# LeonOrou/OPF-Graph-Neural-Solver

Measured on AMD Instinct MI355X. Metric: grids/sec (fwd+bwd) on batched case118, K=4, higher is better.
Workload: dtype f32

## Files before the change

### opf-graph-neural-solver_amd/csrc/gns_backward_split.hip

```cpp
#include "gns_device.h"
#include "gns_kernels.h"
#include "gns_dw.h"
#include "gns_phys_device.h"

typedef int gns_i8v __attribute__((ext_vector_type(8)));
#ifndef GNS_BWDS_ONE_LAYOUT
#define GNS_BWDS_ONE_LAYOUT 0
#endif
#ifndef GNS_BWDS_WPE
#define GNS_BWDS_WPE 2
#endif
#ifndef GNS_BWDS_KEEP_SLOPES
#define GNS_BWDS_KEEP_SLOPES 1
#endif
#if GNS_BWDS_KEEP_SLOPES
#define GNS_SLOPES(sl) sl
#define GNS_SLOPE_OF(sl, layer, act, u) sl[layer][u]
#else
#define GNS_SLOPES(sl) nullptr
#define GNS_SLOPE_OF(sl, layer, act, u) dlrelu2(act[u])
#endif
#ifndef GNS_BWDS_FRESH_INPUTS
#define GNS_BWDS_FRESH_INPUTS 1
#endif
#define GNS_BWDS_PHYS_THREADS (GNS_BWDS_PHYS_WAVES * 64)

__global__ void __launch_bounds__(GNS_BWDS_PHYS_THREADS) gns_bwds_phys_kernel(GnsBwdsArgs A) {
  extern __shared__ __attribute__((aligned(16))) float lds[];
  constexpr int W = GNS_BWDS_PHYS_WAVES;
  const int lane = threadIdx.x & 63;
  const int wave = __builtin_amdgcn_readfirstlane(threadIdx.x >> 6);
  const int N = A.N, E = A.E, K = A.K, k = A.k;
  cip topo = (cip)A.topo;
  const long long g = blockIdx.x;
  long long b = g * GNS_LANES + lane;
  bool live = b < A.Bt;
  if (A.group_topo) {
    const int s = A.slot_grid[g * GNS_LANES + lane];
    b = s;
    live = s >= 0 && s < A.Bt;
    if (!gns_group_topo(A.topo, A.group_topo, g, N, E, topo)) return;
  }
  constexpr int pidx = 4;
  static_assert(GNS_BWDS_PHYS_WAVES == 16, "pidx");
  const cip in_ptr = topo + topo[TH_IN_PTR], out_ptr = topo + topo[TH_OUT_PTR], q2p = topo + topo[TH_Q2P], is_gen = topo + topo[TH_IS_GEN],
            incd_ptr = topo + topo[TH_INCD_PTR], incd = topo + topo[TH_INCD],
            part = topo + topo[TH_PART] + pidx * (GNS_MAXP + 1), epart = topo + topo[TH_EPART] + pidx * (GNS_MAXP + 1);
  const int n0 = part[wave], n1 = part[wave + 1];
  const int e0 = epart[wave], e1 = epart[wave + 1];
  const bool use_plane = A.use_plane != 0, plane_dp = A.use_plane == 2;
  float* const red = lds;
  float* const pl_v = lds + W * GNS_LANES;
  float* const pl_th = pl_v + (use_plane ? N * GNS_LANES : 0);
  float* const pl_dp = pl_th + (plane_dp ? N * GNS_LANES : 0);
  const long long R = gns_in_rows(N, E);
  const float* IN = A.in;
  const long long in_base = g * R, row_ein = in_base + 3LL * N, row_eout = row_ein + 3LL * E, row_grid = row_eout + E;
  const float gt = (live && A.g_total) ? A.g_total[b] : 0.f;
  const float gl = (live && A.g_last) ? A.g_last[b] : 0.f;
  const int RB = A.RB, RBA = A.RBA;
  auto state_row = [&](int slot, int n) { return (((long long)slot * A.G + g) * N + n) * RB; };
  auto adj_row = [&](int n) { return (g * N + n) * RBA; };
  auto slot_ptr = [&](int j, int p) { return A.slots + ((g * 6 + j) * E + p) * GNS_LANES + lane; };
  const f4 gsum = *row_ptr(IN, row_grid, lane);
  const float invN = 1.0f / (float)N;
  const bool last = k == K - 1;
  const int mode = A.mode;
  const bool x2_live = mode == 2 || k + 1 < K - 1;
  const float cdp = 2.f * (gt * A.gwk + (last ? gl : 0.f)) * invN;
  const f2 lamv = reinterpret_cast<const f2*>(A.lam)[((long long)k * A.G + g) * GNS_LANES + lane];
  const int bits = (int)lamv.y;
  const bool low1 = bits & 1, low2 = bits & 2;

  float lb = 0.f;
  constexpr int PB = 4;
  for (int nb = n0; nb < n1; nb += PB) {
    f4 s1[PB], a0[PB], x0[PB], x1[PB], x2[PB], b1[PB];
#pragma unroll
    for (int j = 0; j < PB; ++j) {
      const int n = min(nb + j, n1 - 1);
      const long long ar = adj_row(n);
      s1[j] = *row_ptr(A.state, state_row(k + 1, n), lane);
      b1[j] = *row_ptr(IN, in_base + 3LL * n + 1, lane);
      if (!last) {
        a0[j] = *row_ptr(A.adj, ar, lane);
        x0[j] = *row_ptr(A.adj, ar + (mode == 2 ? 3 : 1), lane);
        x1[j] = *row_ptr(A.adj, ar + (mode == 0 ? 2 : (mode == 2 ? 3 : 1)), lane);
        x2[j] = *row_ptr(A.adj, ar + (x2_live ? 3 : 1), lane);
      }
    }
#pragma unroll
    for (int j = 0; j < PB; ++j) {
      const int n = nb + j;
      if (n < n1) {
        f4 a;
        if (last) {
          const float vb = (live && A.g_v) ? ((s1[j].x < 0.f) ? 0.f : A.g_v[b * N + n]) : 0.f;
          const float tb = (live && A.g_theta) ? A.g_theta[b * N + n] : 0.f;
          a = f4{vb, tb, 0.f, 0.f};
        } else {
          f4 xs;
          if (mode == 2) xs = x2[j];
          else if (mode == 1) xs = x2_live ? f4{x2[j].x + x0[j].x, x2[j].y + x0[j].y, x2[j].z + x0[j].z, 0.f} : x0[j];
          else if (x2_live) xs = f4{(x2[j].x + x0[j].x) + x1[j].x, (x2[j].y + x0[j].y) + x1[j].y, (x2[j].z + x0[j].z) + x1[j].z, 0.f};
          else xs = f4{x0[j].x + x1[j].x, x0[j].y + x1[j].y, x0[j].z + x1[j].z, 0.f};
          a = f4{a0[j].x + xs.x, a0[j].y + xs.y, xs.z, 0.f};
        }
        a.z = a.z + cdp * s1[j].z;
        a.w = 2.f * b1[j].w * s1[j].x;
        *row_ptr(A.adj, adj_row(n), lane) = a;
        if (use_plane) { pl_v[n * GNS_LANES + lane] = s1[j].x; pl_th[n * GNS_LANES + lane] = s1[j].y; }
        if (plane_dp) pl_dp[n * GNS_LANES + lane] = a.z;
        lb += a.z * (low2 ? 2.f * (b1[j].y - b1[j].x) : 2.f * (b1[j].z - b1[j].y));
      }
    }
  }
  red[wave * GNS_LANES + lane] = lb;
  __syncthreads();
  float lbar = 0.f;
#pragma unroll
  for (int w = 0; w < W; ++w) lbar += red[w * GNS_LANES + lane];
  const float pgbar = lbar / (low1 ? 2.f * (gsum.y - gsum.z) : 2.f * (gsum.w - gsum.y));

  {
    const cip erec = topo + topo[TH_EREC];
    struct EdgeIn { f4 e1v, o0; float vs, ths, vt, tht, tha, thb, thc, thd, Fb, Tb; bool gs, gt; };
    auto edge_load = [&](int p, EdgeIn& L) {
      const gns_i8v r = *reinterpret_cast<const __attribute__((address_space(4))) gns_i8v*>(erec + 8 * p);
      const int s = r[0], t = r[1], ia = r[2], ib = r[3], q = r[4], ic = r[5], id = r[6];
      L.gs = is_gen[s] != 0; L.gt = is_gen[t] != 0;
      L.e1v = *row_ptr(IN, row_ein + 3LL * p + 1, lane);
      L.o0 = *row_ptr(IN, row_eout + q, lane);
      if (use_plane) {
        L.vs = pl_v[s * GNS_LANES + lane]; L.ths = pl_th[s * GNS_LANES + lane];
        L.vt = pl_v[t * GNS_LANES + lane]; L.tht = pl_th[t * GNS_LANES + lane];
        L.tha = pl_th[ia * GNS_LANES + lane]; L.thb = pl_th[ib * GNS_LANES + lane];
        L.thc = pl_th[ic * GNS_LANES + lane]; L.thd = pl_th[id * GNS_LANES + lane];
        if (plane_dp) { L.Fb = pl_dp[t * GNS_LANES + lane]; L.Tb = pl_dp[s * GNS_LANES + lane]; }
        else { L.Fb = row_ptr(A.adj, adj_row(t), lane)->z; L.Tb = row_ptr(A.adj, adj_row(s), lane)->z; }
      } else {
        const f4 ss = *row_ptr(A.state, state_row(k + 1, s), lane), st = *row_ptr(A.state, state_row(k + 1, t), lane);
        L.vs = ss.x; L.ths = ss.y; L.vt = st.x; L.tht = st.y;
        L.tha = row_ptr(A.state, state_row(k + 1, ia), lane)->y; L.thb = row_ptr(A.state, state_row(k + 1, ib), lane)->y;
        L.thc = row_ptr(A.state, state_row(k + 1, ic), lane)->y; L.thd = row_ptr(A.state, state_row(k + 1, id), lane)->y;
        L.Fb = row_ptr(A.adj, adj_row(t), lane)->z;
        L.Tb = row_ptr(A.adj, adj_row(s), lane)->z;
      }
    };
    auto edge_adjoint = [&](int p, const EdgeIn& L) {
      const LineTrig T = line_trig<false>(L.ths, L.tht, L.tha, L.thb, L.thc, L.thd, L.e1v.w, L.o0.z);
      const LineAdj R = line_state_adjoint(T, L.vs, L.vt, L.e1v.y, L.e1v.z, L.o0.x, L.o0.y, L.Fb, L.Tb, pgbar);
      if (!L.gs) *slot_ptr(0, p) = R.dvs;
      if (!L.gt) *slot_ptr(1, p) = R.dvt;
      *slot_ptr(2, p) = R.dths;
      *slot_ptr(4, p) = R.dbar; *slot_ptr(5, p) = R.dbar2;
    };
    for (int p = e0; p < e1; p += 2) {
      EdgeIn L0, L1;
      edge_load(p, L0);
      edge_load(min(p + 1, e1 - 1), L1);
      edge_adjoint(p, L0);
      if (p + 1 < e1) edge_adjoint(p + 1, L1);
    }
  }
  __syncthreads();

  for (int n = n0; n < n1; ++n) {
    const long long ar = adj_row(n);
    const f4 a0 = *row_ptr(A.adj, ar, lane);
    float vbar = a0.x, thbar = a0.y;
    const float dpb = a0.z;
    const int p0 = in_ptr[n], p1 = in_ptr[n + 1], q0 = out_ptr[n], q1 = out_ptr[n + 1], i0 = incd_ptr[n], i1 = incd_ptr[n + 1];
    const bool gen = is_gen[n] != 0;
    {
      float ai[4], bi[4], ao[4], bo[4], ci[8];
#pragma unroll
// ... 77 lines not shown
  f32x4 T1[NB1], T2, T4[NT4];
  cfp nb, ptl;

  __device__ __forceinline__ void init(const GnsBwdsArgs& A) {
    const long long koff = A.k;
    nb = (cfp)A.pn + A.n_off[C::NPHI + l] + koff * A.n_sz[C::NPHI + l];
    ptl = (cfp)A.pt + A.t_off[C::NPHI + l] + koff * A.t_sz[C::NPHI + l];
    scalar_cache_warm(ptl, A.t_sz[C::NPHI + l]);
#if !GNS_BWDS_ONE_LAYOUT
    scalar_cache_warm(nb, A.n_sz[C::NPHI + l]);
#endif
    const f32x4 z4 = {0.f, 0.f, 0.f, 0.f};
#pragma unroll
    for (int t = 0; t < NB1; ++t) T1[t] = z4;
#pragma unroll
    for (int t = 0; t < NT4; ++t) T4[t] = z4;
    T2 = z4;
  }

  template <bool ACC_GS, bool STEP0, bool IG = false>
  __device__ __forceinline__ void bus(const GnsBwdsArgs& A, float* rec, int lane, long long g, int n, float g3s, f2 (&xs)[XL],
                                      f2 (&macc)[D / 2], f4& xsum, f2 (&gS)[H / 2]) {
    f2 (&S)[H / 2] = reinterpret_cast<f2 (&)[H / 2]>(xs[SOFF]);
    load_pairs<H>(A.msg, ((((long long)A.k * A.G + g) * A.N + n) * C::NPHI + fphi) * C::HQ, lane, S);
    WFirst wf;
    f2 a1[H / 2], a2[H / 2], g2[H / 2], g1[H / 2];
    f2 sl[2][H / 2];
    using TL [[maybe_unused]] = TLay<LIN, H, OUTP>;
#if GNS_BWDS_ONE_LAYOUT
    (void)wf;
    mlp2_fwd<LIN, H>(ptl, xs, a1, a2, NoBG{}, NoLink{}, GNS_SLOPES(sl));
#else
    using LKm = std::conditional_t<STEP0, NoLink, L2>; using LKs = std::conditional_t<STEP0, std::conditional_t<FOLD4, L0, NoLink>, std::conditional_t<FOLD4, L1, L2>>;
    if constexpr (STEP0) {
      f2 u4[H / 2];
      const f2 (&st)[2] = reinterpret_cast<const f2 (&)[2]>(xs[0]);
      const f2 (&tl)[(LIN - 4 - D + 1) / 2] = reinterpret_cast<const f2 (&)[(LIN - 4 - D + 1) / 2]>(xs[SOFF]);
      phi_head<4, H>(ptl, st, u4);
      phi_tail<LIN, H, 4 + D>(ptl, u4, tl, a1, a2, NoBG{}, NoLink{}, GNS_SLOPES(sl));
    } else {
      mlp2_fwd<LIN, H>(ptl, xs, a1, a2, NoBG{}, L0{nullptr, nb, &wf}, GNS_SLOPES(sl));
    }
#endif
#if GNS_BWDS_ONE_LAYOUT
    if constexpr (l == 2) {
      bwd_rows_fwd_layout<H, OUTP>(ptl + TL::oW4, macc, g2);
    } else {
      const f2 g3v[1] = {f2{g3s, 0.f}};
      bwd_rows_fwd_layout<H, 2>(ptl + TL::oW4, g3v, g2);
    }
#else
    if constexpr (l == 2) {
      bwd_rows<OUTP, H>(nb, macc, g2, NoBG{}, LKm{&wf, nullptr, nullptr});
    } else {
      const f2 g3v[1] = {f2{g3s, 0.f}};
      bwd_rows<2, H>(nb, g3v, g2, NoBG{}, LKs{&wf, nb + NL::oW2, &wf});
    }
#endif
#pragma unroll
    for (int u = 0; u < H / 2; ++u) g2[u] = g2[u] * GNS_SLOPE_OF(sl, 1, a2, u);
    if constexpr (FOLD4 || FOLDM) {
      static_for<0, H / 2>([&](auto j_) { constexpr int j = decltype(j_)::value; gws_putB<SW>(rec, lane, 8 + j, a2[j]); });
      gws_putB<SW>(rec, lane, 8 + H / 2, f2{1.f, 0.f});
      if constexpr (FOLDM) {
        static_for<0, 8>([&](auto j_) { constexpr int j = decltype(j_)::value; gws_putA<SW>(rec, lane, j, macc[j]); });
        gws_w2r(); gws_pass<SW, 16>(rec, lane, T4[0]); gws_r2w();
      }
    } else {
      static_for<0, H / 2>([&](auto j_) { constexpr int j = decltype(j_)::value; gws_putB<SW>(rec, lane, j, a2[j]); });
      gws_putB<SW>(rec, lane, H / 2, f2{1.f, 0.f});
      static_for<0, NA4>([&](auto t_) {
        constexpr int t = decltype(t_)::value;
        if constexpr (l == 2) {
          static_for<0, 6>([&](auto j_) { constexpr int j = decltype(j_)::value; if constexpr (6 * t + j < D / 2) gws_putA<SW>(rec, lane, j, macc[6 * t + j]); });
        } else {
          gws_putA<SW>(rec, lane, 0, f2{g3s, 0.f});
        }
        gws_w2r(); gws_pass<SW>(rec, lane, T4[t]); gws_r2w();
      });
    }
#if GNS_BWDS_ONE_LAYOUT
    bwd_rows_fwd_layout<H, H>(ptl + TL::oW2, g2, g1);
#else
    bwd_rows<H, H>(nb + NL::oW2, g2, g1, NoBG{}, std::conditional_t<FOLD4, L2, NoLink>{&wf, nullptr, nullptr});
#endif
#pragma unroll
    for (int u = 0; u < H / 2; ++u) g1[u] = g1[u] * GNS_SLOPE_OF(sl, 0, a1, u);
    if constexpr (IG && STEP0) {
      float ax[4];
#pragma unroll
      for (int i = 0; i < 4; ++i) {
        float acc = 0.f;
#pragma unroll
        for (int u = 0; u < H / 2; ++u) { acc = fmaf(ptl[i * H + 2 * u], g1[u].x, acc); acc = fmaf(ptl[i * H + 2 * u + 1], g1[u].y, acc); }
        ax[i] = acc;
      }
      xsum.x += ax[0]; xsum.y += ax[1]; xsum.z += ax[2]; xsum.w += ax[3];
    }
    static_for<0, H / 2>([&](auto j_) { constexpr int j = decltype(j_)::value; gws_putA<SW>(rec, lane, j, g2[j]); gws_putB<SW>(rec, lane, j, a1[j]); });
    gws_putB<SW>(rec, lane, H / 2, f2{1.f, 0.f});
    gws_w2r(); gws_pass<SW>(rec, lane, T2); gws_r2w();
    static_for<0, H / 2>([&](auto j_) { constexpr int j = decltype(j_)::value; gws_putA<SW>(rec, lane, j, g1[j]); });
    if constexpr (FOLD4) gws_putA<SW>(rec, lane, H / 2, f2{g3s, 0.f});
    if constexpr (FOLDM) static_for<0, (OUT - 16) / 2>([&](auto j_) { constexpr int j = decltype(j_)::value; gws_putA<SW>(rec, lane, H / 2 + j, macc[8 + j]); });
    static_for<0, NB1>([&](auto t_) {
      constexpr int t = decltype(t_)::value;
      constexpr int po = (WIDE && t == NB1 - 1) ? W2OFF / 2 : 0;
      static_for<0, 8>([&](auto j_) { constexpr int j = decltype(j_)::value; if constexpr (8 * t + j < XL) gws_putB<SW>(rec, lane, po + j, xs[8 * t + j]); });
      gws_w2r(); gws_pass<SW, (WIDE && t == NB1 - 1) ? W2OFF : 0>(rec, lane, T1[t]); gws_r2w();
    });
    auto to_consumers = [&](auto ip_, f2 v) {
      constexpr int ip = decltype(ip_)::value;
      if constexpr (ip == 0) { xsum.x += v.x; xsum.y += v.y; }
      else if constexpr (ip == 1) xsum.z += v.x;
      else if constexpr (ip < SOFF) macc[ip - 2] += v;
      else if constexpr (ip < SOFF + H / 2) { if constexpr (ACC_GS) gS[ip - SOFF] += v; else gS[ip - SOFF] = v; }
    };
#if GNS_BWDS_ONE_LAYOUT
    bwd_from_fwd_layout<2 * (SOFF + H / 2), H, cf16p>(ptl, g1, to_consumers);
#else
    if constexpr (STEP0) {
      constexpr int G0 = (2 * SOFF) / 4, G1 = (2 * SOFF + H - 1) / 4 + 1;
      bwd_inputs<G1 - G0, H>(nb + NL::total + G0 * H * 4, g1, [&](auto ip_, f2 v) {
        constexpr int ip = decltype(ip_)::value + 2 * G0;
        if constexpr (ip >= SOFF && ip < SOFF + H / 2) { if constexpr (ACC_GS) gS[ip - SOFF] += v; else gS[ip - SOFF] = v; }
      });
    } else {
      bwd_inputs<(LIN + 3) / 4, H>(nb + NL::total, g1, to_consumers);
    }
#endif
  }

  __device__ __forceinline__ void flush(const GnsBwdsArgs& A, int lane, float* slab) {
    const long long koff = A.k;
    constexpr int ob1 = LIN * H, oW2 = ob1 + H, ob2 = oW2 + H * H, oW4 = ob2 + H, ob4 = oW4 + OUT * H;
    float* lb_ = slab + A.g_off[C::NPHI + l] + koff * A.g_sz[C::NPHI + l];
    static_for<0, NB1>([&](auto t_) { constexpr int t = decltype(t_)::value;
      gws_flush(lane, T1[t], lb_, [&](int c, int il) {
        const bool lastw = WIDE && t == NB1 - 1;
        const int i = 16 * t + il;
        if (c < H) return (lastw && il >= XT) ? -1 : (i < LIN ? c * LIN + i : (i == LIN ? ob1 + c : -1));
        if (FOLD4 && lastw && c == H && il >= XT && il <= XT + H) return il - XT < H ? oW4 + (il - XT) : ob4;
        if (FOLDM && lastw && c >= H && c < H + (OUT - 16) && il >= XT && il <= XT + H) { const int j = 16 + c - H; return il - XT < H ? oW4 + j * H + (il - XT) : ob4 + j; }
        return -1; }, true); });
    gws_flush(lane, T2, lb_, [&](int c, int il) { return c < H ? (il < H ? oW2 + c * H + il : (il == H ? ob2 + c : -1)) : -1; }, true);
    if constexpr (FOLDM)
      gws_flush(lane, T4[0], lb_, [&](int c, int il) { return il < H ? oW4 + c * H + il : (il == H ? ob4 + c : -1); }, true);
    else if constexpr (!FOLD4)
    static_for<0, NA4>([&](auto t_) { constexpr int t = decltype(t_)::value;
      gws_flush(lane, T4[t], lb_, [&](int c, int il) { const int j = 12 * t + c; return (c < 12 && j < OUT) ? (il < H ? oW4 + j * H + il : (il == H ? ob4 + j : -1)) : -1; }, true); });
  }
};

template <int D, int H, bool MULTI, int PF>
struct BwdsPhi : BwdsShape<D, H, MULTI> {
  using B = BwdsShape<D, H, MULTI>;
  using C = typename B::C;
  using SW = typename B::SW;
  using L0 = typename B::L0; using L2 = typename B::L2;
  static constexpr int XL = B::XL, PIN = B::PIN, NDM = B::NDM, NDMF = B::NDMF;
  static constexpr bool WIDE = B::WIDE;

  f32x4 TP1, TP2, TPm[NDMF];
  cfp pnb, ptb;

  __device__ __forceinline__ void init(const GnsBwdsArgs& A) {
    const long long koff = A.k;
    pnb = (cfp)A.pn + A.n_off[PF] + koff * A.n_sz[PF];
    ptb = (cfp)A.pt + A.t_off[PF] + koff * A.t_sz[PF];
    scalar_cache_warm(ptb, A.t_sz[PF]);
#if !GNS_BWDS_ONE_LAYOUT
    scalar_cache_warm(pnb, A.n_sz[PF]);
#endif
    const f32x4 z4 = {0.f, 0.f, 0.f, 0.f};
#pragma unroll
    for (int t = 0; t < NDMF; ++t) TPm[t] = z4;
    TP1 = z4; TP2 = z4;
  }

  template <bool STEP0, bool IG = false>
  __device__ __forceinline__ void bus(const GnsBwdsArgs& A, float* rec, int lane, const f2 (&xs)[XL], const f2 (&gS)[H / 2],
                                      f2 (&macc)[D / 2], int p0, int p1, long long row_ein) {
    if (p0 >= p1) return;
    const float* IN = A.in;
    const f2 (&m)[D / 2] = reinterpret_cast<const f2 (&)[D / 2]>(xs[2]);
    WFirst wf;
    (void)wf;
    f2 uh[H / 2], G1[H / 2];
    if constexpr (WIDE)
      static_for<0, (D - 16) / 2>([&](auto j_) { constexpr int j = decltype(j_)::value; gws_putB<SW>(rec, lane, 8 + (PIN - D + 2) / 2 + j, m[8 + j]); });
    if constexpr (STEP0) {
#pragma unroll
      for (int j = 0; j < H / 2; ++j) uh[j] = f2{0.f, 0.f};
    } else {
      phi_head<D, H>(ptb, m, uh);
    }
#pragma unroll
    for (int j = 0; j < H / 2; ++j) G1[j] = f2{0.f, 0.f};
    for (int p = p0; p < p1; ++p) {
      const f4 ea = *row_ptr(IN, row_ein + 3LL * p, lane), eb = *row_ptr(IN, row_ein + 3LL * p + 1, lane);
      const f2 xt[3] = {f2{ea.x, ea.y}, f2{ea.z, ea.w}, f2{eb.x, 0.f}};
      f2 a1[H / 2], a2[H / 2], g2[H / 2], g1[H / 2];
      f2 sl[2][H / 2];
#if GNS_BWDS_ONE_LAYOUT
      phi_tail<PIN, H, D>(ptb, uh, xt, a1, a2, NoBG{}, NoLink{}, GNS_SLOPES(sl));
#pragma unroll
      for (int u = 0; u < H / 2; ++u) g2[u] = gS[u] * GNS_SLOPE_OF(sl, 1, a2, u);
      bwd_rows_fwd_layout<H, H>(ptb + TLay2<PIN, H>::oW2, g2, g1);
#else
      phi_tail<PIN, H, D>(ptb, uh, xt, a1, a2, NoBG{}, L0{nullptr, pnb, &wf}, GNS_SLOPES(sl));
#pragma unroll
      for (int u = 0; u < H / 2; ++u) g2[u] = gS[u] * GNS_SLOPE_OF(sl, 1, a2, u);
      bwd_rows<H, H>(pnb, g2, g1, NoBG{}, L2{&wf, nullptr, nullptr});
#endif
#pragma unroll
      for (int u = 0; u < H / 2; ++u) { g1[u] = g1[u] * GNS_SLOPE_OF(sl, 0, a1, u); G1[u] += g1[u]; }
      if constexpr (IG) {
        float fa[5];
#pragma unroll
        for (int f = 0; f < 5; ++f) {
          float acc = 0.f;
#pragma unroll
          for (int u = 0; u < H / 2; ++u) { acc = fmaf(ptb[(D + f) * H + 2 * u], g1[u].x, acc); acc = fmaf(ptb[(D + f) * H + 2 * u + 1], g1[u].y, acc); }
          fa[f] = acc;
        }
        f4* r0 = row_ptr(A.igrad, row_ein + 3LL * p, lane);
        f4* r1 = row_ptr(A.igrad, row_ein + 3LL * p + 1, lane);
        const f4 o0 = *r0, o1 = *r1;
        *r0 = f4{o0.x + fa[0], o0.y + fa[1], o0.z + fa[2], o0.w + fa[3]};
        *r1 = f4{o1.x + fa[4], o1.y, o1.z, o1.w};
      }
      constexpr int pw = WIDE ? 8 : 0;
      static_for<0, H / 2>([&](auto j_) { constexpr int j = decltype(j_)::value; gws_putA<SW>(rec, lane, j, g1[j]); });
      gws_putB<SW>(rec, lane, pw + 0, xt[0]); gws_putB<SW>(rec, lane, pw + 1, xt[1]); gws_putB<SW>(rec, lane, pw + 2, f2{xt[2].x, 1.f});
      gws_w2r(); gws_pass<SW, 2 * pw>(rec, lane, TP1); gws_r2w();
      static_for<0, H / 2>([&](auto j_) { constexpr int j = decltype(j_)::value; gws_putA<SW>(rec, lane, j, g2[j]); gws_putB<SW>(rec, lane, j, a1[j]); });
      gws_putB<SW>(rec, lane, H / 2, f2{1.f, 0.f});
      gws_w2r(); gws_pass<SW>(rec, lane, TP2); gws_r2w();
    }
    if constexpr (STEP0) return;
#if GNS_BWDS_ONE_LAYOUT
    bwd_from_fwd_layout<D, H, cf16p>(ptb, G1, [&](auto ip_, f2 v) { macc[decltype(ip_)::value] += v; });
#else
    bwd_inputs<(D + 3) / 4, H>(pnb + NLay2<PIN, H>::total, G1, [&](auto ip_, f2 v) {
      constexpr int ip = decltype(ip_)::value;
      if constexpr (ip < D / 2) macc[ip] += v;
    });
#endif
    static_for<0, H / 2>([&](auto j_) { constexpr int j = decltype(j_)::value; gws_putA<SW>(rec, lane, j, G1[j]); });
    static_for<0, NDMF>([&](auto t_) {
      constexpr int t = decltype(t_)::value;
      static_for<0, 8>([&](auto j_) { constexpr int j = decltype(j_)::value; if constexpr (8 * t + j < D / 2) gws_putB<SW>(rec, lane, j, m[8 * t + j]); });
      gws_w2r(); gws_pass<SW>(rec, lane, TPm[t]); gws_r2w();
    });
  }

  __device__ __forceinline__ void flush(const GnsBwdsArgs& A, int lane, float* slab) {
    const long long koff = A.k;
    constexpr int pb1 = PIN * H, pW2 = pb1 + H, pb2 = pW2 + H * H;
    float* pb_ = slab + A.g_off[PF] + koff * A.g_sz[PF];
    gws_flush(lane, TP1, pb_, [&](int c, int il) {
      if (c >= H) return -1;
      if (il < PIN - D) return c * PIN + D + il;
      if (il == PIN - D) return pb1 + c;
      if (WIDE && il >= PIN - D + 1 && il < PIN - D + 1 + (D - 16)) return c * PIN + 16 + (il - (PIN - D + 1));
      return -1; }, true);
    gws_flush(lane, TP2, pb_, [&](int c, int il) { return c < H ? (il < H ? pW2 + c * H + il : (il == H ? pb2 + c : -1)) : -1; }, true);
    static_for<0, NDMF>([&](auto t_) { constexpr int t = decltype(t_)::value;
      gws_flush(lane, TPm[t], pb_, [&](int c, int il) { const int i = 16 * t + il; return (c < H && i < D) ? c * PIN + i : -1; }, true); });
  }
};

template <int D, int H, bool MULTI, int FAMS, bool STEP0, bool GROUPED, bool IG>
__global__ void __launch_bounds__(64) __attribute__((amdgpu_waves_per_eu(GNS_BWDS_WPE))) gns_bwds_sweep_kernel(GnsBwdsArgs A) {
  using C = GnsDims<D, H, MULTI>;
  static_assert(MULTI || FAMS == 7, "the single phi is reversed after all three L nets");
  constexpr int RB = C::RB, MQ = C::MQ, RBA = 4 + 6 * MQ;
  constexpr bool HAS_T = FAMS & 1, HAS_V = FAMS & 2, HAS_M = FAMS & 4;
  constexpr int SLOT = HAS_M ? 2 : (HAS_T ? 0 : 1);
  constexpr int LIN = C::LF_IN, XL = (LIN + 1) / 2;
  constexpr int RECF = 64 * (D > 16 ? GwSubWide::RS : GwSub::RS);
  __shared__ __attribute__((aligned(16))) float rec[RECF];
  const int lane = threadIdx.x;
  const long long GB = (A.G + A.R - 1) / A.R;
  const long long bid = blockIdx.x;
  const long long gb = bid % GB;
  const int c = (int)(bid / GB);
  const int N = A.N, E = A.E, K = A.K, k = A.k;
  cip topo = (cip)A.topo;
  cip part = topo + topo[TH_PART] + A.part_idx * (GNS_MAXP + 1), in_ptr = topo + topo[TH_IN_PTR], is_gen = topo + topo[TH_IS_GEN];
  int n0 = part[c], n1 = part[c + 1];
  const long long g0 = gb * A.R, g1 = (g0 + A.R < A.G) ? g0 + A.R : A.G;
  float* slab = A.slab + (gb * A.C + c) * A.slab_floats;
  const bool lastk = k == K - 1;
  if (HAS_M && lastk) {
    float* z0 = slab + A.g_off[C::NPHI + 2] + (long long)(K - 1) * A.g_sz[C::NPHI + 2];
    for (int i = lane; i < (int)A.g_sz[C::NPHI + 2]; i += 64) z0[i] = 0.f;
    if constexpr (MULTI) {
      float* z1 = slab + A.g_off[2] + (long long)(K - 1) * A.g_sz[2];
      for (int i = lane; i < (int)A.g_sz[2]; i += 64) z1[i] = 0.f;
    }
    if (!HAS_T && !HAS_V) return;
  }
  BwdsL<D, H, MULTI, 2> lm;
  BwdsL<D, H, MULTI, 0> lt;
  BwdsL<D, H, MULTI, 1> lv;
  BwdsPhi<D, H, MULTI, MULTI ? 2 : 0> pm;
  BwdsPhi<D, H, MULTI, MULTI ? 1 : 0> pt;
  BwdsPhi<D, H, MULTI, 0> pv;
  if constexpr (HAS_M) { lm.init(A); pm.init(A); }
  if constexpr (HAS_T) { lt.init(A); if constexpr (MULTI) pt.init(A); }
  if constexpr (HAS_V) { lv.init(A); if constexpr (MULTI) pv.init(A); }
  constexpr bool step0 = STEP0;
  const int par = k & 1, parn = par ^ 1;
  const bool m2_live = (A.mode == 2) || k + 1 < K - 1;
  const long long R = gns_in_rows(N, E);

  for (long long g = g0; g < g1; ++g) {
    if constexpr (GROUPED) {
      if (!gns_group_topo(A.topo, A.group_topo, g, N, E, topo)) continue;
      part = topo + topo[TH_PART] + A.part_idx * (GNS_MAXP + 1); in_ptr = topo + topo[TH_IN_PTR]; is_gen = topo + topo[TH_IS_GEN];
      n0 = part[c]; n1 = part[c + 1];
    }
    const long long row_ein = g * R + 3LL * N;
    auto state_row = [&](int slot, int n) { return (((long long)slot * A.G + g) * N + n) * RB; };
    for (int n = n0; n < n1; ++n) {
      const long long ar = (g * N + n) * RBA, rr = state_row(k, n);
      const f4 a0 = *row_ptr(A.adj, ar, lane);
      const f4 s0 = *row_ptr(A.state, rr, lane);
      f2 xs[XL];
      f2 (&m)[D / 2] = reinterpret_cast<f2 (&)[D / 2]>(xs[2]);
      load_pairs<D>(A.state, (step0 ? state_row(0, n0) : rr) + 1, lane, m);
      f2 macc[D / 2];
      if (HAS_M && !lastk) {
        const long long mr = ar + 4 + (long long)parn * 3 * MQ;
        if (A.mode == 2) {
          load_pairs<D>(A.adj, mr + 2 * MQ, lane, macc);
        } else {
          f2 p0v[D / 2];
          load_pairs<D>(A.adj, mr, lane, p0v);
          load_pairs<D>(A.adj, mr + (m2_live ? 2 : 0) * MQ, lane, macc);
          if (A.mode == 0) {
            f2 p1v[D / 2];
            load_pairs<D>(A.adj, mr + MQ, lane, p1v);
#pragma unroll
            for (int i = 0; i < D / 2; ++i) macc[i] = m2_live ? (macc[i] + p0v[i]) + p1v[i] : p0v[i] + p1v[i];
          } else {
#pragma unroll
            for (int i = 0; i < D / 2; ++i) macc[i] = m2_live ? macc[i] + p0v[i] : p0v[i];
          }
        }
      } else {
#pragma unroll
        for (int i = 0; i < D / 2; ++i) macc[i] = f2{0.f, 0.f};
      }
      f4 xsum = f4{0.f, 0.f, 0.f, 0.f};
      const int p0 = in_ptr[n], p1 = in_ptr[n + 1];
      xs[0] = f2{s0.x, s0.y}; xs[1] = f2{s0.z, s0.w};
      xs[XL - 1] = f2{(float)(p1 - p0), 1.f};
      f2 gS[H / 2];
      const float g3v = is_gen[n] ? 0.f : a0.x;
      auto fresh = [&]() {
#if GNS_BWDS_FRESH_INPUTS
        pin_all(xs);
#endif
      };
      if constexpr (MULTI) {
        if constexpr (HAS_M) { if (!lastk) { fresh(); lm.template bus<false, STEP0, IG>(A, rec, lane, g, n, 0.f, xs, macc, xsum, gS); fresh(); pm.template bus<STEP0, IG>(A, rec, lane, xs, gS, macc, p0, p1, row_ein); } }
        if constexpr (HAS_T) { fresh(); lt.template bus<false, STEP0, IG>(A, rec, lane, g, n, a0.y, xs, macc, xsum, gS); fresh(); pt.template bus<STEP0, IG>(A, rec, lane, xs, gS, macc, p0, p1, row_ein); }
        if constexpr (HAS_V) { if (!is_gen[n]) { fresh(); lv.template bus<false, STEP0, IG>(A, rec, lane, g, n, g3v, xs, macc, xsum, gS); fresh(); pv.template bus<STEP0, IG>(A, rec, lane, xs, gS, macc, p0, p1, row_ein); } }
      } else {
#pragma unroll
        for (int j = 0; j < H / 2; ++j) gS[j] = f2{0.f, 0.f};
        if (!lastk) { fresh(); lm.template bus<true, STEP0, IG>(A, rec, lane, g, n, 0.f, xs, macc, xsum, gS); }
        fresh(); lt.template bus<true, STEP0, IG>(A, rec, lane, g, n, a0.y, xs, macc, xsum, gS);
        if (!is_gen[n]) { fresh(); lv.template bus<true, STEP0, IG>(A, rec, lane, g, n, g3v, xs, macc, xsum, gS); }
        fresh(); pm.template bus<STEP0, IG>(A, rec, lane, xs, gS, macc, p0, p1, row_ein);
      }
      if constexpr (!step0) {
        *row_ptr(A.adj, ar + 1 + SLOT, lane) = xsum;
        store_pairs<D>(A.adj, ar + 4 + (par * 3 + SLOT) * MQ, lane, macc);
      } else if constexpr (IG) {
        *row_ptr(A.adj, ar + 1 + SLOT, lane) = xsum;
      }
    }
  }
  if constexpr (HAS_M) { if (!lastk) lm.flush(A, lane, slab); if (MULTI ? !lastk : true) pm.flush(A, lane, slab); }
  if constexpr (HAS_T) { lt.flush(A, lane, slab); if constexpr (MULTI) pt.flush(A, lane, slab); }
  if constexpr (HAS_V) { lv.flush(A, lane, slab); if constexpr (MULTI) pv.flush(A, lane, slab); }
}

__global__ void __launch_bounds__(GNS_BWDS_PHYS_THREADS) gns_bwds_igrad_phys_kernel(GnsBwdsArgs A) {
  __shared__ float red[GNS_BWDS_PHYS_WAVES * GNS_LANES];
  constexpr int W = GNS_BWDS_PHYS_WAVES;
  const int lane = threadIdx.x & 63;
  const int wave = __builtin_amdgcn_readfirstlane(threadIdx.x >> 6);
  const int N = A.N, E = A.E, k = A.k;
  cip topo = (cip)A.topo;
  const long long g = blockIdx.x;
  constexpr int pidx = 4;
  const cip in_ptr = topo + topo[TH_IN_PTR], out_ptr = topo + topo[TH_OUT_PTR], q2p = topo + topo[TH_Q2P], is_gen = topo + topo[TH_IS_GEN],
            part = topo + topo[TH_PART] + pidx * (GNS_MAXP + 1), epart = topo + topo[TH_EPART] + pidx * (GNS_MAXP + 1);
  const int n0 = part[wave], n1 = part[wave + 1];
  const int e0 = epart[wave], e1 = epart[wave + 1];
  const long long R = gns_in_rows(N, E);
  const float* IN = A.in;
  float* IG = A.igrad;
  const long long in_base = g * R, row_ein = in_base + 3LL * N, row_eout = row_ein + 3LL * E, row_grid = row_eout + E;
  const int RB = A.RB, RBA = A.RBA;
  auto state_row = [&](int n) { return (((long long)(k + 1) * A.G + g) * N + n) * RB; };
  auto adj_row = [&](int n) { return (g * N + n) * RBA; };
  auto slot_ptr = [&](int j, int p) { return A.slots + ((g * 6 + j) * E + p) * GNS_LANES + lane; };
  const f4 gsum = *row_ptr(IN, row_grid, lane);
  const f2 lamv = reinterpret_cast<const f2*>(A.lam)[((long long)k * A.G + g) * GNS_LANES + lane];
  const float lam = lamv.x;
  const int bits = (int)lamv.y;
  const bool low1 = bits & 1, low2 = bits & 2;

  float lb = 0.f;
  for (int n = n0; n < n1; ++n) {
    const float dpb = row_ptr(A.adj, adj_row(n), lane)->z;
    const f4 b1 = *row_ptr(IN, in_base + 3LL * n + 1, lane);
    lb += dpb * (low2 ? 2.f * (b1.y - b1.x) : 2.f * (b1.z - b1.y));
  }
  red[wave * GNS_LANES + lane] = lb;
  __syncthreads();
  float lbar = 0.f;
#pragma unroll
  for (int w = 0; w < W; ++w) lbar += red[w * GNS_LANES + lane];
  const float pgbar = lbar / (low1 ? 2.f * (gsum.y - gsum.z) : 2.f * (gsum.w - gsum.y));

  for (int n = n0; n < n1; ++n) {
    const float dpb = row_ptr(A.adj, adj_row(n), lane)->z;
    const float v = row_ptr(A.state, state_row(n), lane)->x;
    f4* r0 = row_ptr(IG, in_base + 3LL * n, lane);
    f4* r1 = row_ptr(IG, in_base + 3LL * n + 1, lane);
    const f4 o0 = *r0, o1 = *r1;
    *r0 = f4{o0.x - dpb, o0.y, o0.z + (pgbar - dpb) * (v * v), o0.w};
    const f4 dpg = low2 ? f4{dpb * (1.f - 2.f * lam), dpb * (2.f * lam), 0.f, 0.f}
                        : f4{0.f, dpb * (2.f - 2.f * lam), dpb * (2.f * lam - 1.f), 0.f};
    *r1 = f4{o1.x + dpg.x, o1.y + dpg.y, o1.z + dpg.z, o1.w};
  }
  if (wave == 0) {
    f4* rg = row_ptr(IG, row_grid, lane);
    const f4 o = *rg;
    const f4 d = low1 ? f4{pgbar, pgbar * (-2.f * lam), pgbar * (2.f * lam - 1.f), 0.f}
                      : f4{pgbar, pgbar * (2.f * lam - 2.f), 0.f, pgbar * (1.f - 2.f * lam)};
    *rg = f4{o.x + d.x, o.y + d.y, o.z + d.z, o.w + d.w};
  }

  const cip erec = topo + topo[TH_EREC];
  for (int p = e0; p < e1; ++p) {
    const gns_i8v r = *reinterpret_cast<const __attribute__((address_space(4))) gns_i8v*>(erec + 8 * p);
    const int s = r[0], t = r[1], ia = r[2], ib = r[3], q = r[4], ic = r[5], id = r[6];
    const f4 e1v = *row_ptr(IN, row_ein + 3LL * p + 1, lane);
    const f4 o0 = *row_ptr(IN, row_eout + q, lane);
    const f4 ss = *row_ptr(A.state, state_row(s), lane), st = *row_ptr(A.state, state_row(t), lane);
    const float vs = ss.x, ths = ss.y, vt = st.x, tht = st.y;
    const float tha = row_ptr(A.state, state_row(ia), lane)->y, thb = row_ptr(A.state, state_row(ib), lane)->y;
    const float thc = row_ptr(A.state, state_row(ic), lane)->y, thd = row_ptr(A.state, state_row(id), lane)->y;
    const float Fb = row_ptr(A.adj, adj_row(t), lane)->z, Tb = row_ptr(A.adj, adj_row(s), lane)->z;
    const LineTrig T = line_trig<false>(ths, tht, tha, thb, thc, thd, e1v.w, o0.z);
    const LinePro Q = line_prologue(T, vs, vt, e1v.y, e1v.z, o0.x, o0.y, pgbar);
    const LineParAdj dP = line_param_adjoint(T, Q, vs, vt, e1v.z, o0.y, Fb, Tb);
    f4* rs = row_ptr(IG, row_ein + 3LL * p + 1, lane);
    f4* rt = row_ptr(IG, row_eout + q, lane);
    const f4 os = *rs, ot = *rt;
    *rs = f4{os.x, os.y + dP.ybs, os.z + dP.tbs, os.w + dP.sbs};
    *rt = f4{ot.x + dP.ybt, ot.y + dP.tbt, ot.z + dP.sbt, ot.w};
    const bool gs = is_gen[s] != 0, gt = is_gen[t] != 0;
    if (gs || gt) {
      const LineAdj R = line_state_adjoint(T, Q, vs, vt, e1v.y, o0.x, Fb, Tb);
      if (gs) *slot_ptr(0, p) = R.dvs;
      if (gt) *slot_ptr(1, p) = R.dvt;
    }
  }
  __syncthreads();
  for (int n = n0; n < n1; ++n) {
    if (!is_gen[n]) continue;
    float dv = 0.f;
    for (int p = in_ptr[n]; p < in_ptr[n + 1]; ++p) dv += *slot_ptr(1, p);
    for (int qq = out_ptr[n]; qq < out_ptr[n + 1]; ++qq) dv += *slot_ptr(0, q2p[qq]);
    f4* r2 = row_ptr(IG, in_base + 3LL * n + 2, lane);
    const f4 o2 = *r2;
    *r2 = f4{o2.x, o2.y, o2.z + dv, o2.w};
  }
}

__global__ void __launch_bounds__(64) gns_bwds_igrad_unpack_kernel(GnsBwdsArgs A, const float* __restrict__ buses, const float* __restrict__ lines,
                                                                   const float* __restrict__ gens, int Gn, float* __restrict__ gbu,
                                                                   float* __restrict__ gli, float* __restrict__ gge) {
  const int lane = threadIdx.x;
  const long long g = blockIdx.x;
  const int u = blockIdx.y;
  const int N = A.N, E = A.E, K = A.K;
  const long long b = g * GNS_LANES + lane;
  if (b >= A.Bt) return;
  cip topo = (cip)A.topo;
  const long long R = gns_in_rows(N, E);
  const float* IG = A.igrad;
  const long long in_base = g * R, row_ein = in_base + 3LL * N, row_eout = row_ein + 3LL * E, row_grid = row_eout + E;
  const f4 gs = *row_ptr(IG, row_grid, lane);
  if (u < N) {
    const int n = u;
    const long long ar = (g * N + n) * A.RBA;
    const f4 a0 = *row_ptr(A.adj, ar, lane);
    const int mode = A.mode;
    const bool x2_live = mode == 2 || 0 < K - 1;
    const f4 x0 = *row_ptr(A.adj, ar + 1, lane), x1 = *row_ptr(A.adj, ar + 2, lane), x2 = *row_ptr(A.adj, ar + 3, lane);
    f4 xs;
    if (mode == 2) xs = x2;
    else if (mode == 1) xs = x2_live ? x2 + x0 : x0;
    else xs = x2_live ? (x2 + x0) + x1 : x0 + x1;
    const f4 r0 = *row_ptr(IG, in_base + 3LL * n, lane), r1 = *row_ptr(IG, in_base + 3LL * n + 1, lane),
             r2 = *row_ptr(IG, in_base + 3LL * n + 2, lane);
    const float* bu = buses + b * (long long)N * 6 + n * 6;
    const float* ge = gens + b * (long long)Gn * 7;
    const float Gs = bu[4], Bs = bu[5];
    const int q0 = topo[topo[TH_GEN_PTR] + n], q1 = topo[topo[TH_GEN_PTR] + n + 1];
    float vg = 0.f;
    for (int q = q0; q < q1; ++q) vg += ge[topo[topo[TH_GEN_IDX] + q] * 7 + 4];
    const float v0 = (vg == 0.f) ? 1.f : vg;
    const float dp0b = xs.z, dq0b = xs.w;
    const float v0b = a0.x + xs.x + r2.z - 2.f * Gs * v0 * dp0b + 2.f * Bs * v0 * dq0b;
    const float vgb = (vg == 0.f) ? 0.f : v0b;
    if (gbu) {
      float* o = gbu + b * (long long)N * 6 + n * 6;
      o[2] += (r0.x + gs.x) - dp0b;
      o[3] += r0.y - dq0b;
      o[4] += r0.z - dp0b * (v0 * v0);
      o[5] += r0.w + dq0b * (v0 * v0);
    }
    if (gge) {
      for (int q = q0; q < q1; ++q) {
        float* o = gge + b * (long long)Gn * 7 + topo[topo[TH_GEN_IDX] + q] * 7;
        o[1] += r1.z + gs.w;
        o[2] += r1.x + gs.z;
        o[3] += r1.y + gs.y;
        o[4] += vgb;
        o[5] += dq0b;
        o[6] += dp0b;
      }
    }
    return;
  }
  const int p = u - N;
  if (p >= E || !gli) return;
  const int e = topo[topo[TH_IN_EID] + p];
  const f4 f0 = *row_ptr(IG, row_ein + 3LL * p, lane), f1 = *row_ptr(IG, row_ein + 3LL * p + 1, lane);
  float yb = 0.f, tb = 0.f, sb = 0.f;
  if (e < N) {
    const cip out_ptr = topo + topo[TH_OUT_PTR], in_ptr = topo + topo[TH_IN_PTR], q2p = topo + topo[TH_Q2P], p2q = topo + topo[TH_P2Q];
    for (int q = out_ptr[e]; q < out_ptr[e + 1]; ++q) { const f4 s = *row_ptr(IG, row_ein + 3LL * q2p[q] + 1, lane); yb += s.y; tb += s.z; sb += s.w; }
    for (int pp = in_ptr[e]; pp < in_ptr[e + 1]; ++pp) { const f4 t = *row_ptr(IG, row_eout + p2q[pp], lane); yb += t.x; tb += t.y; sb += t.z; }
  }
  const float* li = lines + b * (long long)E * 7 + e * 7;
  const float r = li[2], x = li[3];
  const float y = __fdiv_rn(1.0f, __fsqrt_rn(__fadd_rn(__fmul_rn(r, r), __fmul_rn(x, x))));
  const float y3 = y * y * y;
  float* o = gli + b * (long long)E * 7 + e * 7;
  o[2] += f0.x - r * y3 * yb;
  o[3] += f0.y - x * y3 * yb;
  o[4] += f0.z;
  o[5] += f0.w + tb;
  o[6] += f1.x + sb;
}

int gns_launch_bwds_igrad_phys(const GnsBwdsArgs& A, hipStream_t st) {
  hipLaunchKernelGGL(gns_bwds_igrad_phys_kernel, dim3((unsigned)A.G), dim3(GNS_BWDS_PHYS_THREADS), 0, st, A);
  return hipGetLastError() == hipSuccess ? GNS_OK : GNS_ELAUNCH;
}

int gns_launch_bwds_igrad_unpack(const GnsBwdsArgs& A, const float* buses, const float* lines, const float* gens, int Gn,
                                 float* grad_buses, float* grad_lines, float* grad_gens, hipStream_t st) {
  hipLaunchKernelGGL(gns_bwds_igrad_unpack_kernel, dim3((unsigned)A.G, (unsigned)(A.N + A.E)), dim3(64), 0, st, A, buses, lines, gens, Gn,
                     grad_buses, grad_lines, grad_gens);
  return hipGetLastError() == hipSuccess ? GNS_OK : GNS_ELAUNCH;
}

int gns_bwds_supported(int d, int h, int multi) {
  (void)multi;
#define GNS_CASE(DD, HH) if (d == DD && h == HH) return 1;
  GNS_FOR_EACH_DIMS(GNS_CASE)
#undef GNS_CASE
  return 0;
}

size_t gns_bwds_phys_lds(int N, int* use_plane) {
  const size_t red = (size_t)GNS_BWDS_PHYS_WAVES * GNS_LANES * 4;
  const size_t plane = (size_t)N * GNS_LANES * 4;
  const int level = red + 3 * plane <= (size_t)160 * 1024 ? 2 : (red + 2 * plane <= (size_t)160 * 1024 ? 1 : 0);
  if (use_plane) *use_plane = level;
  return red + (level == 2 ? 3 : (level == 1 ? 2 : 0)) * plane;
}

int gns_launch_bwds_phys(const GnsBwdsArgs& A, size_t lds, hipStream_t st) {
  hipLaunchKernelGGL(gns_bwds_phys_kernel, dim3((unsigned)A.G), dim3(GNS_BWDS_PHYS_THREADS), lds, st, A);
  return hipGetLastError() == hipSuccess ? GNS_OK : GNS_ELAUNCH;
}

int gns_launch_bwds_sweep(int d, int h, int multi, const GnsBwdsArgs& A, hipStream_t st) {
  const long long GB = (A.G + A.R - 1) / A.R;
  const unsigned blocks = (unsigned)(GB * A.C);
#define GNS_SWEEP1(DD, HH, MM, FAMS, GR, IG) do { if (A.k == 0) hipLaunchKernelGGL((gns_bwds_sweep_kernel<DD, HH, MM, FAMS, true, GR, IG>), dim3(blocks), dim3(64), 0, st, A); \
                                                 else hipLaunchKernelGGL((gns_bwds_sweep_kernel<DD, HH, MM, FAMS, false, GR, IG>), dim3(blocks), dim3(64), 0, st, A); } while (0)
#define GNS_SWEEP(DD, HH, MM, FAMS) do { if (A.group_topo) GNS_SWEEP1(DD, HH, MM, FAMS, true, false); \
                                         else if (A.igrad) GNS_SWEEP1(DD, HH, MM, FAMS, false, true); \
                                         else GNS_SWEEP1(DD, HH, MM, FAMS, false, false); } while (0)
#define GNS_CASE(DD, HH)                                                                                                    \
  if (d == DD && h == HH) {                                                                                                 \
    if (!multi) { if (A.mode != 2) return GNS_EINVAL; GNS_SWEEP(DD, HH, false, 7); }                                        \
    else if (A.mode == 2) GNS_SWEEP(DD, HH, true, 7);                                                                       \
    else if (A.mode == 1) { GNS_SWEEP(DD, HH, true, 4); GNS_SWEEP(DD, HH, true, 3); }                                       \
    else { GNS_SWEEP(DD, HH, true, 4); GNS_SWEEP(DD, HH, true, 1); GNS_SWEEP(DD, HH, true, 2); }                            \
    return hipGetLastError() == hipSuccess ? GNS_OK : GNS_ELAUNCH;                                                          \
  }
  GNS_FOR_EACH_DIMS(GNS_CASE)
#undef GNS_CASE
#undef GNS_SWEEP
#undef GNS_SWEEP1
  return GNS_EUNSUPPORTED;
}

int gns_bwds_init_device() {
  return hipFuncSetAttribute((const void*)gns_bwds_phys_kernel, hipFuncAttributeMaxDynamicSharedMemorySize, 160 * 1024) == hipSuccess
             ? GNS_OK : GNS_ELAUNCH;
}
```

Measured before the change: 5.954 million.

## Prefetch next line rows and next bus state in backward sweep kernel

Adds software prefetching to the backward sweep kernel. The next incident line's input rows are loaded one iteration ahead inside the phi bus loop, and the next bus's adjacency and state rows are requested before the current bus's phi work, so global-load latency is hidden behind compute. The prefetching only applies to the shape selected by a specialization predicate (multi, D=20, H=10, families 3 and 4). It also adds a disabled-by-default option that folds the last-k M zeroing into the T sweep and skips the M sweep launch. The extra in-flight values raise register pressure, which could lower occupancy.

```diff
diff --git a/opf-graph-neural-solver_amd/csrc/gns_backward_split.hip b/opf-graph-neural-solver_amd/csrc/gns_backward_split.hip
--- a/opf-graph-neural-solver_amd/csrc/gns_backward_split.hip
+++ b/opf-graph-neural-solver_amd/csrc/gns_backward_split.hip
@@ -22,6 +22,24 @@
 #endif
 #ifndef GNS_BWDS_FRESH_INPUTS
 #define GNS_BWDS_FRESH_INPUTS 1
+#endif
+#ifndef GNS_BWDS_LINE_AHEAD
+#define GNS_BWDS_LINE_AHEAD 1
+#endif
+#ifndef GNS_BWDS_BUS_AHEAD
+#define GNS_BWDS_BUS_AHEAD 1
+#endif
+#ifndef GNS_BWDS_AH_M
+#define GNS_BWDS_AH_M 5
+#endif
+#ifndef GNS_BWDS_AH_M0
+#define GNS_BWDS_AH_M0 5
+#endif
+#ifndef GNS_BWDS_AH_T0
+#define GNS_BWDS_AH_T0 4
+#endif
+#ifndef GNS_BWDS_LASTK_FOLD
+#define GNS_BWDS_LASTK_FOLD 0
 #endif
 #define GNS_BWDS_PHYS_THREADS (GNS_BWDS_PHYS_WAVES * 64)
 
@@ -405,6 +423,11 @@
   }
 };
 
+struct BwdsLineRows { f4 a, b; };
+__device__ __forceinline__ BwdsLineRows bwds_line_rows(const float* IN, long long row_ein, int p, int lane) {
+  return BwdsLineRows{*row_ptr(IN, row_ein + 3LL * p, lane), *row_ptr(IN, row_ein + 3LL * p + 1, lane)};
+}
+
 template <int D, int H, bool MULTI, int PF>
 struct BwdsPhi : BwdsShape<D, H, MULTI> {
   using B = BwdsShape<D, H, MULTI>;
@@ -431,9 +454,9 @@
     TP1 = z4; TP2 = z4;
   }
 
-  template <bool STEP0, bool IG = false>
+  template <bool STEP0, bool IG = false, bool LA = false>
   __device__ __forceinline__ void bus(const GnsBwdsArgs& A, float* rec, int lane, const f2 (&xs)[XL], const f2 (&gS)[H / 2],
-                                      f2 (&macc)[D / 2], int p0, int p1, long long row_ein) {
+                                      f2 (&macc)[D / 2], int p0, int p1, long long row_ein, const BwdsLineRows& first) {
     if (p0 >= p1) return;
     const float* IN = A.in;
     const f2 (&m)[D / 2] = reinterpret_cast<const f2 (&)[D / 2]>(xs[2]);
@@ -450,8 +473,16 @@
     }
 #pragma unroll
     for (int j = 0; j < H / 2; ++j) G1[j] = f2{0.f, 0.f};
+    f4 ca, cb;
+    if constexpr (LA) { ca = first.a; cb = first.b; }
     for (int p = p0; p < p1; ++p) {
-      const f4 ea = *row_ptr(IN, row_ein + 3LL * p, lane), eb = *row_ptr(IN, row_ein + 3LL * p + 1, lane);
+      f4 na, nb, ea, eb;
+      if constexpr (LA) {
+        na = *row_ptr(IN, row_ein + 3LL * min(p + 1, p1 - 1), lane); nb = *row_ptr(IN, row_ein + 3LL * min(p + 1, p1 - 1) + 1, lane);
+        ea = ca; eb = cb;
+      } else {
+        ea = *row_ptr(IN, row_ein + 3LL * p, lane); eb = *row_ptr(IN, row_ein + 3LL * p + 1, lane);
+      }
       const f2 xt[3] = {f2{ea.x, ea.y}, f2{ea.z, ea.w}, f2{eb.x, 0.f}};
       f2 a1[H / 2], a2[H / 2], g2[H / 2], g1[H / 2];
       f2 sl[2][H / 2];
@@ -490,6 +521,7 @@
       static_for<0, H / 2>([&](auto j_) { constexpr int j = decltype(j_)::value; gws_putA<SW>(rec, lane, j, g2[j]); gws_putB<SW>(rec, lane, j, a1[j]); });
       gws_putB<SW>(rec, lane, H / 2, f2{1.f, 0.f});
       gws_w2r(); gws_pass<SW>(rec, lane, TP2); gws_r2w();
+      if constexpr (LA) { ca = na; cb = nb; }
     }
     if constexpr (STEP0) return;
 #if GNS_BWDS_ONE_LAYOUT
@@ -522,6 +554,19 @@
     static_for<0, NDMF>([&](auto t_) { constexpr int t = decltype(t_)::value;
       gws_flush(lane, TPm[t], pb_, [&](int c, int il) { const int i = 16 * t + il; return (c < H && i < D) ? c * PIN + i : -1; }, true); });
   }
+};
+
+template <int D, int H, bool MULTI, int FAMS, bool GROUPED, bool IG>
+struct BwdsMeasured { static constexpr bool value = MULTI && D == 20 && H == 10 && (FAMS == 3 || FAMS == 4) && !GROUPED && !IG; };
+template <int D>
+struct BwdsTop { f4 a0, s0; f2 m[D / 2], q0[D / 2], q2[D / 2]; };
+template <int D, int H, bool MULTI, int FAMS, bool STEP0, bool GROUPED, bool IG>
+struct BwdsAhead {
+#if GNS_BWDS_BUS_AHEAD
+  static constexpr int value = !BwdsMeasured<D, H, MULTI, FAMS, GROUPED, IG>::value ? 0 : (FAMS == 4 ? (STEP0 ? GNS_BWDS_AH_M0 : GNS_BWDS_AH_M) : (STEP0 ? GNS_BWDS_AH_T0 : 0));
+#else
+  static constexpr int value = 0;
+#endif
 };
 
 template <int D, int H, bool MULTI, int FAMS, bool STEP0, bool GROUPED, bool IG>
@@ -546,7 +591,9 @@
   const long long g0 = gb * A.R, g1 = (g0 + A.R < A.G) ? g0 + A.R : A.G;
   float* slab = A.slab + (gb * A.C + c) * A.slab_floats;
   const bool lastk = k == K - 1;
-  if (HAS_M && lastk) {
+  constexpr bool LA = BwdsMeasured<D, H, MULTI, FAMS, GROUPED, IG>::value && (GNS_BWDS_LINE_AHEAD == 1 || (GNS_BWDS_LINE_AHEAD == 2 && FAMS == 4));
+  constexpr bool ZERO_M = HAS_M || (GNS_BWDS_LASTK_FOLD && MULTI && HAS_T && !GROUPED && !IG);
+  if (ZERO_M && lastk) {
     float* z0 = slab + A.g_off[C::NPHI + 2] + (long long)(K - 1) * A.g_sz[C::NPHI + 2];
     for (int i = lane; i < (int)A.g_sz[C::NPHI + 2]; i += 64) z0[i] = 0.f;
     if constexpr (MULTI) {
@@ -577,13 +624,27 @@
     }
     const long long row_ein = g * R + 3LL * N;
     auto state_row = [&](int slot, int n) { return (((long long)slot * A.G + g) * N + n) * RB; };
+    constexpr int AH = BwdsAhead<D, H, MULTI, FAMS, STEP0, GROUPED, IG>::value;
+    auto request = [&](int nn, BwdsTop<D>& t) {
+      const long long arn = (g * N + nn) * RBA, mrn = arn + 4 + (long long)parn * 3 * MQ;
+      if constexpr (AH & 4) { t.a0 = *row_ptr(A.adj, arn, lane); t.s0 = *row_ptr(A.state, state_row(k, nn), lane); }
+      if constexpr (AH & 2) load_pairs<D>(A.state, state_row(k, nn) + 1, lane, t.m);
+      if constexpr (AH & 1) { load_pairs<D>(A.adj, mrn, lane, t.q0); load_pairs<D>(A.adj, mrn + (m2_live ? 2 : 0) * MQ, lane, t.q2); }
+    };
+    BwdsTop<D> nx;
+    if constexpr (AH != 0) { if (n0 < n1) request(n0, nx); }
     for (int n = n0; n < n1; ++n) {
       const long long ar = (g * N + n) * RBA, rr = state_row(k, n);
-      const f4 a0 = *row_ptr(A.adj, ar, lane);
-      const f4 s0 = *row_ptr(A.state, rr, lane);
+      const f4 a0 = [&]() { if constexpr (AH & 4) return nx.a0; else return *row_ptr(A.adj, ar, lane); }();
+      const f4 s0 = [&]() { if constexpr (AH & 4) return nx.s0; else return *row_ptr(A.state, rr, lane); }();
       f2 xs[XL];
       f2 (&m)[D / 2] = reinterpret_cast<f2 (&)[D / 2]>(xs[2]);
-      load_pairs<D>(A.state, (step0 ? state_row(0, n0) : rr) + 1, lane, m);
+      if constexpr (AH & 2) {
+#pragma unroll
+        for (int i = 0; i < D / 2; ++i) m[i] = nx.m[i];
+      } else {
+        load_pairs<D>(A.state, (step0 ? state_row(0, n0) : rr) + 1, lane, m);
+      }
       f2 macc[D / 2];
       if (HAS_M && !lastk) {
         const long long mr = ar + 4 + (long long)parn * 3 * MQ;
@@ -591,8 +652,13 @@
           load_pairs<D>(A.adj, mr + 2 * MQ, lane, macc);
         } else {
           f2 p0v[D / 2];
-          load_pairs<D>(A.adj, mr, lane, p0v);
-          load_pairs<D>(A.adj, mr + (m2_live ? 2 : 0) * MQ, lane, macc);
+          if constexpr (AH & 1) {
+#pragma unroll
+            for (int i = 0; i < D / 2; ++i) { p0v[i] = nx.q0[i]; macc[i] = nx.q2[i]; }
+          } else {
+            load_pairs<D>(A.adj, mr, lane, p0v);
+            load_pairs<D>(A.adj, mr + (m2_live ? 2 : 0) * MQ, lane, macc);
+          }
           if (A.mode == 0) {
             f2 p1v[D / 2];
             load_pairs<D>(A.adj, mr + MQ, lane, p1v);
@@ -607,6 +673,7 @@
 #pragma unroll
         for (int i = 0; i < D / 2; ++i) macc[i] = f2{0.f, 0.f};
       }
+      auto ahead = [&]() { if constexpr (AH != 0) request(min(n + 1, n1 - 1), nx); };
       f4 xsum = f4{0.f, 0.f, 0.f, 0.f};
       const int p0 = in_ptr[n], p1 = in_ptr[n + 1];
       xs[0] = f2{s0.x, s0.y}; xs[1] = f2{s0.z, s0.w};
@@ -618,17 +685,19 @@
         pin_all(xs);
 #endif
       };
+      BwdsLineRows lr;
+      auto first = [&]() { if constexpr (LA) lr = bwds_line_rows(A.in, row_ein, max(min(p0, E - 1), 0), lane); };
       if constexpr (MULTI) {
-        if constexpr (HAS_M) { if (!lastk) { fresh(); lm.template bus<false, STEP0, IG>(A, rec, lane, g, n, 0.f, xs, macc, xsum, gS); fresh(); pm.template bus<STEP0, IG>(A, rec, lane, xs, gS, macc, p0, p1, row_ein); } }
-        if constexpr (HAS_T) { fresh(); lt.template bus<false, STEP0, IG>(A, rec, lane, g, n, a0.y, xs, macc, xsum, gS); fresh(); pt.template bus<STEP0, IG>(A, rec, lane, xs, gS, macc, p0, p1, row_ein); }
-        if constexpr (HAS_V) { if (!is_gen[n]) { fresh(); lv.template bus<false, STEP0, IG>(A, rec, lane, g, n, g3v, xs, macc, xsum, gS); fresh(); pv.template bus<STEP0, IG>(A, rec, lane, xs, gS, macc, p0, p1, row_ein); } }
+        if constexpr (HAS_M) { if (!lastk) { first(); fresh(); lm.template bus<false, STEP0, IG>(A, rec, lane, g, n, 0.f, xs, macc, xsum, gS); ahead(); fresh(); pm.template bus<STEP0, IG, LA>(A, rec, lane, xs, gS, macc, p0, p1, row_ein, lr); } }
+        if constexpr (HAS_T) { first(); fresh(); lt.template bus<false, STEP0, IG>(A, rec, lane, g, n, a0.y, xs, macc, xsum, gS); if constexpr (!HAS_M) ahead(); fresh(); pt.template bus<STEP0, IG, LA>(A, rec, lane, xs, gS, macc, p0, p1, row_ein, lr); }
+        if constexpr (HAS_V) { if (!is_gen[n]) { first(); fresh(); lv.template bus<false, STEP0, IG>(A, rec, lane, g, n, g3v, xs, macc, xsum, gS); fresh(); pv.template bus<STEP0, IG, LA>(A, rec, lane, xs, gS, macc, p0, p1, row_ein, lr); } }
       } else {
 #pragma unroll
         for (int j = 0; j < H / 2; ++j) gS[j] = f2{0.f, 0.f};
         if (!lastk) { fresh(); lm.template bus<true, STEP0, IG>(A, rec, lane, g, n, 0.f, xs, macc, xsum, gS); }
-        fresh(); lt.template bus<true, STEP0, IG>(A, rec, lane, g, n, a0.y, xs, macc, xsum, gS);
+        first(); fresh(); lt.template bus<true, STEP0, IG>(A, rec, lane, g, n, a0.y, xs, macc, xsum, gS);
         if (!is_gen[n]) { fresh(); lv.template bus<true, STEP0, IG>(A, rec, lane, g, n, g3v, xs, macc, xsum, gS); }
-        fresh(); pm.template bus<STEP0, IG>(A, rec, lane, xs, gS, macc, p0, p1, row_ein);
+        fresh(); pm.template bus<STEP0, IG, LA>(A, rec, lane, xs, gS, macc, p0, p1, row_ein, lr);
       }
       if constexpr (!step0) {
         *row_ptr(A.adj, ar + 1 + SLOT, lane) = xsum;
@@ -855,6 +924,7 @@
 int gns_launch_bwds_sweep(int d, int h, int multi, const GnsBwdsArgs& A, hipStream_t st) {
   const long long GB = (A.G + A.R - 1) / A.R;
   const unsigned blocks = (unsigned)(GB * A.C);
+  const bool fold_m = GNS_BWDS_LASTK_FOLD && A.k == A.K - 1 && !A.group_topo && !A.igrad;
 #define GNS_SWEEP1(DD, HH, MM, FAMS, GR, IG) do { if (A.k == 0) hipLaunchKernelGGL((gns_bwds_sweep_kernel<DD, HH, MM, FAMS, true, GR, IG>), dim3(blocks), dim3(64), 0, st, A); \
                                                  else hipLaunchKernelGGL((gns_bwds_sweep_kernel<DD, HH, MM, FAMS, false, GR, IG>), dim3(blocks), dim3(64), 0, st, A); } while (0)
 #define GNS_SWEEP(DD, HH, MM, FAMS) do { if (A.group_topo) GNS_SWEEP1(DD, HH, MM, FAMS, true, false); \
@@ -864,8 +934,8 @@
   if (d == DD && h == HH) {                                                                                                 \
     if (!multi) { if (A.mode != 2) return GNS_EINVAL; GNS_SWEEP(DD, HH, false, 7); }                                        \
     else if (A.mode == 2) GNS_SWEEP(DD, HH, true, 7);                                                                       \
-    else if (A.mode == 1) { GNS_SWEEP(DD, HH, true, 4); GNS_SWEEP(DD, HH, true, 3); }                                       \
-    else { GNS_SWEEP(DD, HH, true, 4); GNS_SWEEP(DD, HH, true, 1); GNS_SWEEP(DD, HH, true, 2); }                            \
+    else if (A.mode == 1) { if (!fold_m) GNS_SWEEP(DD, HH, true, 4); GNS_SWEEP(DD, HH, true, 3); }                          \
+    else { if (!fold_m) GNS_SWEEP(DD, HH, true, 4); GNS_SWEEP(DD, HH, true, 1); GNS_SWEEP(DD, HH, true, 2); }               \
     return hipGetLastError() == hipSuccess ? GNS_OK : GNS_ELAUNCH;                                                          \
   }
   GNS_FOR_EACH_DIMS(GNS_CASE)
```

Measured after the change: 6.042 million, median of 6. 1.01x the previous value.
